# kaist-ina/stellatrain

Measured on AMD Instinct MI355X. Metric: grad-codec GB/s (dense fp32 in) per GPU; thresholdv16 k=1% on 64 MiB bucket, higher is better.
Workload: dtype f32; 1 GPU; thresholdv16 k=167772 (1%) on 64 MiB fp32 buckets; step = 64 keys (4096 MiB) per GPU in 16 batched calls of 4, call j on stream j % 4; n=16777216, dst_len=167772, streams=4, parallelism=bucket-sharded x1, no collective

## Files before the change

### include/stg/codec.h

```cpp
#ifndef STG_CODEC_H
#define STG_CODEC_H

#include <stddef.h>
#include <stdint.h>

#ifdef __cplusplus
extern "C" {
#endif

#define STG_OK 0
#define STG_ERR_INVALID (-1)
#define STG_ERR_UNKNOWN (-2)
#define STG_ERR_HIP (-3)
#define STG_ERR_UNSUPPORTED (-4)
#define STG_ERR_DEVICE (-5)

typedef struct stg_codec *stg_codec_t;
typedef struct stg_sgd *stg_sgd_t;
typedef struct stg_adam *stg_adam_t;

int stg_codec_create(const char *method, int device, stg_codec_t *out);
int stg_codec_destroy(stg_codec_t h);
const char *stg_codec_name(stg_codec_t h);

// ... 11 lines not shown
    size_t n;
    uint32_t k;
    uint32_t *d_idx;
    size_t idx_cap;
    float *d_val;
    size_t val_cap;
    int32_t idx_offset;
    uint32_t *d_count;
} stg_bucket_t;

int stg_codec_compress_batch_device(stg_codec_t h, const stg_bucket_t *buckets, size_t nbuckets, void *stream);

int stg_merge_compress_batch_device(stg_codec_t h, const stg_bucket_t *buckets, float *const *d_residuals,
                                    size_t nbuckets, void *stream);

int stg_merge_gather_compress_device(stg_codec_t h, const stg_bucket_t *bucket, float *d_residual,
                                     const float *const *d_grads, int num_gpus, void *stream);

int stg_codec_compress_wire_batch_device(stg_codec_t h, const stg_bucket_t *buckets, const int *flags,
                                         size_t nbuckets, void *stream);

int stg_codec_get_state(stg_codec_t h, const char *key, const void *key_ptr, float *threshold,
                        float *threshold_inc, void *stream);

int stg_codec_set_timing(stg_codec_t h, int enable);
int stg_codec_get_timing(stg_codec_t h, double *ms3, uint64_t *calls);

int stg_codec_debug_words(stg_codec_t h, void *stream, uint32_t *out, int n);

int stg_codec_check(stg_codec_t h);

int stg_scatter_merge_device(const uint32_t *d_idx, const float *d_val, size_t per_rank, int world, size_t n,
                             float *d_dense, uint8_t *d_mark, uint32_t *d_out_idx, float *d_out_val,
                             uint32_t *d_out_count, void *stream);
int stg_scatter_merge_check(void *stream);
int stg_scatter_merge_release(void *stream);

int stg_error_feedback_device(float *d_grad, size_t n, const uint32_t *d_idx, size_t numel, float *d_residual,
                              void *stream);

int stg_sgd_create(int device, float lr, float momentum, float dampening, float weight_decay, int nesterov,
                   int maximize, stg_sgd_t *out);
int stg_sgd_destroy(stg_sgd_t o);
int stg_sgd_optimize_raw_device(stg_sgd_t o, const char *name, float *d_param, uint32_t param_len,
                                const float *d_grad, const uint32_t *d_idx, uint32_t grad_len,
                                const uint32_t *d_grad_len, void *stream);
// ... 86 lines not shown
```

### stellatrain_amd/_capi.py

```python
from __future__ import annotations

import ctypes as C
import os
import re

_HERE = os.path.dirname(os.path.abspath(__file__))
LIB_PATH = os.environ.get("STG_CODEC_LIB") or os.path.join(_HERE, "libstg_codec.so")
HEADER = os.path.join(os.path.dirname(_HERE), "include", "stg", "codec.h")

STG_OK = 0
ERRORS = {-1: "STG_ERR_INVALID", -2: "STG_ERR_UNKNOWN", -3: "STG_ERR_HIP", -4: "STG_ERR_UNSUPPORTED",
          -5: "STG_ERR_DEVICE"}


class CodecError(RuntimeError):

    def __init__(self, code: int, msg: str):
        super().__init__(msg)
        self.code = code


class StgBucket(C.Structure):
    _fields_ = [("key", C.c_char_p), ("d_src", C.c_void_p), ("n", C.c_size_t), ("k", C.c_uint32),
                ("d_idx", C.c_void_p), ("idx_cap", C.c_size_t), ("d_val", C.c_void_p), ("val_cap", C.c_size_t),
# ... 2 lines not shown

class StgRankStream(C.Structure):
    _fields_ = [("d_idx", C.c_void_p), ("d_val", C.c_void_p), ("flag", C.c_int)]


class StgWireRx(C.Structure):
    _fields_ = [("d_idx_in", C.c_void_p), ("d_val_in", C.c_void_p), ("numel", C.c_size_t), ("flag", C.c_int),
                ("d_idx", C.c_void_p), ("d_val", C.c_void_p)]


_lib: C.CDLL | None = None

_SIGS = {
    "stg_codec_create": (C.c_int, [C.c_char_p, C.c_int, C.POINTER(C.c_void_p)]),
    "stg_codec_destroy": (C.c_int, [C.c_void_p]),
    "stg_codec_name": (C.c_char_p, [C.c_void_p]),
    "stg_codec_compress_host": (C.c_int, [C.c_void_p, C.c_char_p, C.c_void_p, C.c_size_t, C.c_uint32, C.c_void_p,
                                          C.c_size_t, C.c_void_p, C.c_size_t, C.c_int32, C.POINTER(C.c_size_t)]),
    "stg_codec_compress_device": (C.c_int, [C.c_void_p, C.c_char_p, C.c_void_p, C.c_size_t, C.c_uint32, C.c_void_p,
                                            C.c_size_t, C.c_void_p, C.c_size_t, C.c_int32, C.c_void_p, C.c_void_p]),
    "stg_codec_compress_batch_device": (C.c_int, [C.c_void_p, C.POINTER(StgBucket), C.c_size_t, C.c_void_p]),
    "stg_codec_get_state": (C.c_int, [C.c_void_p, C.c_char_p, C.c_void_p, C.POINTER(C.c_float),
                                      C.POINTER(C.c_float), C.c_void_p]),
    "stg_codec_check": (C.c_int, [C.c_void_p]),
    "stg_codec_debug_words": (C.c_int, [C.c_void_p, C.c_void_p, C.c_void_p, C.c_int]),
    "stg_codec_set_timing": (C.c_int, [C.c_void_p, C.c_int]),
    "stg_codec_get_timing": (C.c_int, [C.c_void_p, C.POINTER(C.c_double), C.POINTER(C.c_uint64)]),
    "stg_scatter_merge_device": (C.c_int, [C.c_void_p, C.c_void_p, C.c_size_t, C.c_int, C.c_size_t, C.c_void_p,
                                           C.c_void_p, C.c_void_p, C.c_void_p, C.c_void_p, C.c_void_p]),
    "stg_scatter_merge_check": (C.c_int, [C.c_void_p]),
    "stg_scatter_merge_release": (C.c_int, [C.c_void_p]),
    "stg_error_feedback_device": (C.c_int, [C.c_void_p, C.c_size_t, C.c_void_p, C.c_size_t, C.c_void_p, C.c_void_p]),
    "stg_sgd_create": (C.c_int, [C.c_int, C.c_float, C.c_float, C.c_float, C.c_float, C.c_int, C.c_int,
                                 C.POINTER(C.c_void_p)]),
    "stg_sgd_destroy": (C.c_int, [C.c_void_p]),
    "stg_sgd_optimize_raw_device": (C.c_int, [C.c_void_p, C.c_char_p, C.c_void_p, C.c_uint32, C.c_void_p,
                                              C.c_void_p, C.c_uint32, C.c_void_p, C.c_void_p]),
    "stg_sgd_get_momentum": (C.c_int, [C.c_void_p, C.c_char_p, C.c_void_p, C.c_uint32, C.c_void_p]),
    "stg_sgd_set_smart_momentum": (C.c_int, [C.c_void_p, C.c_int]),
    "stg_sgd_get_last": (C.c_int, [C.c_void_p, C.c_char_p, C.c_void_p, C.c_uint32, C.c_void_p]),
    "stg_sgd_get_iter": (C.c_int, [C.c_void_p, C.POINTER(C.c_uint32)]),
    "stg_sgd_check": (C.c_int, [C.c_void_p, C.c_void_p]),
    "stg_merge_optimize_sgd_device": (C.c_int, [C.c_void_p, C.c_char_p, C.c_void_p, C.c_uint32, C.c_void_p,
                                                C.c_void_p, C.c_size_t, C.c_int, C.c_void_p, C.c_void_p,
                                                C.c_void_p, C.c_void_p, C.c_void_p, C.c_void_p]),
    "stg_merge_optimize_adam_device": (C.c_int, [C.c_void_p, C.c_char_p, C.c_void_p, C.c_uint32, C.c_void_p,
# ... 68 lines not shown
```

### stellatrain_amd/compressor.py

```python
from __future__ import annotations

import ctypes as C

import numpy as np

from ._capi import CodecError, StgBucket, check, lib

__all__ = ["Compressor", "ThresholdvCompressor16", "ThresholdvCompressor", "TopkCompressor", "make_compressor",
           "CodecError"]


def _is_torch(x) -> bool:
    return type(x).__module__.startswith("torch")


def _stream_ptr(device: int) -> int:
    import torch
    return torch.cuda.current_stream(device).cuda_stream


class Compressor:

    _method = ""

# ... 131 lines not shown
    def _compress_host(self, name, src, k, dst_idx, dst_val, idx_offset) -> int:
        s = src.numpy() if _is_torch(src) else src
        di = dst_idx.numpy() if _is_torch(dst_idx) else dst_idx
        dv = dst_val.numpy() if _is_torch(dst_val) else dst_val
        if not (isinstance(s, np.ndarray) and s.dtype == np.float32 and s.flags.c_contiguous):
            raise TypeError("src must be a contiguous float32 array/tensor")
        if di.dtype.itemsize != 4 or dv.dtype != np.float32 or not di.flags.c_contiguous or not dv.flags.c_contiguous:
            raise TypeError("dst_idx must be contiguous (u)int32 and dst_val contiguous float32")
        out = C.c_size_t()
        check(lib().stg_codec_compress_host(
            self._h, name.encode(), C.c_void_p(s.ctypes.data), s.size, int(k), C.c_void_p(di.ctypes.data),
            di.size, C.c_void_p(dv.ctypes.data), dv.size, int(idx_offset), C.byref(out)))
        return int(out.value)

    def state(self, name: str = "", key_ptr: int = 0, stream=None):
        t, inc = C.c_float(), C.c_float()
        sp = stream if stream is not None else 0
        rc = lib().stg_codec_get_state(self._h, name.encode(), C.c_void_p(key_ptr), C.byref(t), C.byref(inc),
                                       C.c_void_p(sp))
        if rc != 0:
            return None
        return t.value, inc.value

    def set_timing(self, enable: bool) -> None:
        check(lib().stg_codec_set_timing(self._h, int(enable)))

    def get_timing(self):
        ms = (C.c_double * 3)()
        calls = C.c_uint64()
        check(lib().stg_codec_get_timing(self._h, ms, C.byref(calls)))
        return (ms[0], ms[1], ms[2]), int(calls.value)

    def check_device(self) -> None:
        check(lib().stg_codec_check(self._h))


class ThresholdvCompressor16(Compressor):

    _method = "thresholdv16"

    def __init__(self, thread_pool=None, multicore: bool = True, *, device: int = 0):
        self.multicore_ = multicore
        super().__init__(thread_pool, device=device)


class ThresholdvCompressor(Compressor):
# ... 27 lines not shown
```

### stellatrain_amd/csrc/capi.cpp

```cpp
#include <cmath>
#include <hip/hip_runtime.h>

#include <algorithm>
#include <array>
#include <map>
#include <cstdio>
#include <cstdlib>
#include <cstring>
#include <memory>
#include <mutex>
#include <string>
#include <unordered_map>
#include <vector>

#include <dlfcn.h>

#include "../../include/stg/codec.h"
#include "ws.h"

namespace {

thread_local std::string g_err;

int fail(int code, const std::string &msg) {
// ... 360 lines not shown
        if (lc <= stg::LMAXC && (rc = ws->ensure_lone(lc))) return rc;
    }
    std::array<hipEvent_t, 3> evs{};
    bool timed = false;
    if ((rc = h->take_events(&evs, &timed))) return rc;
    if (++ws->epoch >= (1u << 24)) {
        ws->epoch = 1;
        HIP_TRY(hipMemsetAsync(ws->d.ctl, 0, sizeof(stg::FillCtl), s));
        HIP_TRY(hipMemsetAsync(ws->d.desc, 0, ws->cap_desc * sizeof(stg::ChunkDesc), s));
    }
    stg::Tv16Launch a{};
    a.b = grp.data();
    a.nb = (uint32_t)grp.size();
    a.num_cu = h->num_cu;
    a.ev = timed ? evs.data() : nullptr;
    a.epoch = ws->epoch;
    const uint32_t inflight = fused_inflight();
    constexpr uint32_t XCDS = 8;
    a.max_wg = (uint32_t)(2 * h->num_cu);
    (void)XCDS;
    a.desc_cap = (uint32_t)std::min<size_t>(ws->cap_desc, 0xffffffffu);
    a.lone_cap = (uint32_t)ws->cap_lone;
    a.lone_calls = &ws->lone_calls;
    if (!inflight) {
        HIP_TRY(stg::launch_tv16(a, ws->d, s));
        grp.clear();
        return STG_OK;
    }
    FusedLane &lane = g_lanes[h->device & 63];
    std::lock_guard<std::mutex> lg(lane.mu);
    const size_t max_inflight = inflight;
    while (lane.inflight.size() >= max_inflight) {
        auto old = lane.inflight.front();
        lane.inflight.erase(lane.inflight.begin());
        if (old.second != s) HIP_TRY(hipStreamWaitEvent(s, old.first, 0));
        lane.pool.push_back(old.first);
    }
    HIP_TRY(stg::launch_tv16(a, ws->d, s));
    hipEvent_t done;
    if (!lane.pool.empty()) { done = lane.pool.back(); lane.pool.pop_back(); }
    else HIP_TRY(hipEventCreateWithFlags(&done, hipEventDisableTiming));
    HIP_TRY(hipEventRecord(done, s));
    lane.inflight.emplace_back(done, s);
    grp.clear();
    return STG_OK;
}
// ... 397 lines not shown
        snprintf(b, sizeof b, "device failure flags 0x%x (details: stg_codec_check)", ws->pinned_count[1]);
        return fail(STG_ERR_DEVICE, b);
    }
    *out_count = *ws->pinned_count;
    return STG_OK;
}

int stg_codec_get_state(stg_codec_t h, const char *key, const void *key_ptr, float *threshold, float *threshold_inc,
                        void *stream) {
    if (!h) return fail(STG_ERR_INVALID, "null codec handle");
    HIP_TRY(hipSetDevice(h->device));
    KeyState *st = nullptr;
    {
        std::lock_guard<std::mutex> g(h->mu);
        auto it = h->slot_of.find(state_key(h->method, key, key_ptr));
        if (it == h->slot_of.end()) return fail(STG_ERR_INVALID, "key has no state yet");
        st = h->slot_ptr(it->second);
    }
    HIP_TRY(hipStreamSynchronize(static_cast<hipStream_t>(stream)));
    KeyState hs;
    HIP_TRY(hipMemcpy(&hs, st, sizeof hs, hipMemcpyDeviceToHost));
    if (threshold) *threshold = hs.t;
    if (threshold_inc) *threshold_inc = hs.inc;
    return STG_OK;
}

int stg_codec_set_timing(stg_codec_t h, int enable) {
    if (!h) return fail(STG_ERR_INVALID, "null codec handle");
    std::lock_guard<std::mutex> g(h->mu);
    h->timing = enable != 0;
    return STG_OK;
}

int stg_codec_get_timing(stg_codec_t h, double *ms3, uint64_t *calls) {
    if (!h || !ms3 || !calls) return fail(STG_ERR_INVALID, "null argument");
    HIP_TRY(hipSetDevice(h->device));
    std::lock_guard<std::mutex> g(h->mu);
    for (auto &e : h->ev_pending) {
        HIP_TRY(hipEventSynchronize(e[2]));
        float a = 0, b = 0, c = 0;
        HIP_TRY(hipEventElapsedTime(&a, e[0], e[1]));
        HIP_TRY(hipEventElapsedTime(&b, e[1], e[2]));
        HIP_TRY(hipEventElapsedTime(&c, e[0], e[2]));
        h->ms_acc[0] += a;
        h->ms_acc[1] += b;
        h->ms_acc[2] += c;
// ... 725 lines not shown
```

### stellatrain_amd/csrc/tv16.hip

```cpp
#include <algorithm>
#include <cstdlib>

#include "tv16_dev.h"

namespace stg {

namespace {

using namespace tv16;
constexpr uint32_t kEfAux = 2;

constexpr uint32_t kTv16Ns = 11;
constexpr uint32_t FWG = (kTv16Ns + 1) * 64;
constexpr uint32_t FNW = FWG / 64;
constexpr uint32_t NS = kTv16Ns;
constexpr uint32_t FIN = NS;
static_assert(NS + 1 <= FNW && FWG <= 1024, "streaming group + finisher fit the workgroup");
constexpr uint32_t kTv16Nbuf = 5;
constexpr uint32_t kTv16ScanD = 3;
constexpr uint32_t NBUF = kTv16Nbuf;
constexpr uint32_t CIDR = 2 * NBUF;
constexpr uint32_t kTv16StageB = 72;
constexpr uint32_t kTv16WlB = 64;
constexpr uint32_t STAGE_B = kTv16StageB;
constexpr uint32_t WL_B = kTv16WlB;
constexpr uint32_t kTv16PollSleep = 8;
constexpr uint32_t GB = 512;
constexpr uint32_t SCAN_D_BATCH = kTv16ScanD;
constexpr uint32_t kTv16ScanDLone = 6;
constexpr uint32_t SCAN_D_LONE = kTv16ScanDLone;
constexpr uint32_t MAXG = 512;
__global__ void __launch_bounds__(STG_WG) tv16_seq_sums(const float *__restrict__ src, size_t n,
                                                        float *__restrict__ out, uint32_t nblk) {
    const uint32_t j = blockIdx.x * STG_WG + threadIdx.x;
    if (j >= nblk) return;
    const size_t base = (size_t)j * 16;
    const uint32_t len = (uint32_t)std::min<size_t>(16, n - base);
    float s = 0.f;
    if (len == 16) {
        const float4 *p = reinterpret_cast<const float4 *>(src + base);
        const float4 a = p[0], b = p[1], c = p[2], d = p[3];
        s += fabsf(a.x); s += fabsf(a.y); s += fabsf(a.z); s += fabsf(a.w);
        s += fabsf(b.x); s += fabsf(b.y); s += fabsf(b.z); s += fabsf(b.w);
        s += fabsf(c.x); s += fabsf(c.y); s += fabsf(c.z); s += fabsf(c.w);
        s += fabsf(d.x); s += fabsf(d.y); s += fabsf(d.z); s += fabsf(d.w);
    } else {
// ... 13 lines not shown
struct BucketDesc {
    const float *src;
    uint32_t *idx;
    float *val;
    uint32_t *count_out;
    KeyState *state;
    float *sums_g;
    uint32_t nb, tl, dst_len;
    int32_t idx_offset;
    uint32_t cs, nc;
    float *resid;
    uint32_t wflag, wend;
};

struct BatchArgs {
    BucketDesc bk[MAX_BATCH];
    uint32_t nbk;
    uint32_t epoch;
    uint32_t K;
    FillCtl *ctl;
    ChunkDesc *desc;
    uint32_t *cand;
    uint32_t *fail;
};

struct Lds {
    float4 stage[NBUF][STAGE_B * 4];
    uint32_t stage_line[NBUF][STAGE_B];
    uint64_t wl[NBUF][WL_B];
    uint32_t nst[NBUF];
    uint32_t nwl[NBUF];
    uint32_t qcnt[NBUF];
    uint32_t wcnt[NBUF];
    uint32_t sdone[NBUF];
    float tval[NBUF], incv[NBUF];
    uint32_t cid[CIDR];
    uint32_t cok[CIDR];
    uint32_t mid[CIDR];
    uint32_t fdone;
    uint4 gb[GB];
};
static_assert(sizeof(Lds) <= TV16_SCAN_LDS, "two scan workgroups and a fill workgroup share a CU");

__device__ __forceinline__ constexpr uint32_t spin_site(uint32_t site) { return FAIL_SPIN_TIMEOUT | (1u << (8 + site)); }

struct Ctx {
    const BatchArgs &A;
    Lds &L;
    uint32_t G, w;
    FillCtl *ctlp;
    uint32_t *candp;
    uint32_t *failp;

    __device__ __forceinline__ uint32_t tag(uint32_t kind) const { return (A.epoch << 8) | kind; }
    __device__ __forceinline__ FillCtl *ctl() const { return ctlp; }
    __device__ __forceinline__ CallCtl *cc() const { return &ctlp->cc[A.epoch & 1u]; }
    __device__ __forceinline__ uint32_t *cand(uint32_t b) const { return candp + (size_t)b * CAND_WORDS; }
    __device__ __forceinline__ void fail(uint32_t bits) const { g_or(failp, bits); }
    __device__ __forceinline__ void spin_fail(uint32_t site, uint32_t x0, uint32_t x1, uint32_t x2) const {
        g_or(failp, spin_site(site));
        if (atomicCAS(failp + 1, 0u, site + 1u) == 0u) {
            st_sc1(failp + 2, w);
            st_sc1(failp + 3, x0);
            st_sc1(failp + 4, x1);
            st_sc1(failp + 5, x2);
            st_sc1(failp + 6, A.epoch);
        }
        uint32_t *rec = failp + 8 + 4 * site;
        if (atomicCAS(rec, 0u, w + 1u) == 0u) {
            st_sc1(rec + 1, x0);
            st_sc1(rec + 2, x1);
            st_sc1(rec + 3, x2);
        }
        for (uint32_t b = 0; b < A.nbk; ++b) st_sc1(A.bk[b].count_out, POISON_COUNT);
    }
    __device__ __forceinline__ uint32_t bucket_of(uint32_t k) const {
        uint32_t b = 0;
        while (b + 1 < A.nbk && k >= A.bk[b + 1].cs) ++b;
        return b;
    }
};

constexpr uint32_t TAG_AGG = 1, TAG_DEC = TV16_TAG_DEC;
constexpr uint32_t DEC_B = TV16_DEC_B, DEC_WIN = TV16_DEC_WIN, DEC_TAIL = TV16_DEC_TAIL;
constexpr uint32_t WIN = TV16_WIN;

template <int STAGE, bool EF, uint32_t SCAN_D>
__device__ __forceinline__ void scan_chunk(Ctx &C, uint32_t j, uint32_t k, uint32_t s) {
    Lds &L = C.L;
    const uint32_t par = j % NBUF;
    if (j >= NBUF) {
        uint64_t st2 = 0;
        uint32_t spins = 0;
        for (; lds_ld(&L.fdone) < j + 1 - NBUF; ++spins) {
            __builtin_amdgcn_s_sleep(2);
            if (spin_expired(spins, st2)) { if (flane() == 0) C.spin_fail(1, j, lds_ld(&L.fdone), s); break; }
        }
    }
    const uint32_t b = C.bucket_of(k);
    const BucketDesc &d = C.A.bk[b];
    const uint32_t c = k - d.cs;
    const uint32_t L0 = c * TV16_CHUNK;
    const uint32_t nl = d.nb > L0 ? std::min(TV16_CHUNK, d.nb - L0) : 0u;
    const float t = uni(d.state->t);
    const uint32_t lane = flane(), q = lane & 3;
    if (s == 0 && lane == 0) { L.tval[par] = t; L.incv[par] = uni(d.state->inc); }
    const uint32_t tb = f2u(t);
    const uint32_t wlo = tb > WIN ? tb - WIN : 0u;
    const uint32_t steps = (nl + 15) / 16;
    const uint32_t mine = steps > s ? (steps - s + NS - 1) / NS : 0u;
    uint32_t cnt_w = 0, win_w = 0;
    const __amdgpu_buffer_rsrc_t rsrc = __builtin_amdgcn_make_buffer_rsrc(
        const_cast<float *>(d.src + (size_t)L0 * 16), 0, nl * 64u, 0x00020000);
    const uint32_t lane_line = s * 16 + (lane >> 2);
    const __amdgpu_buffer_rsrc_t rsrc_r = __builtin_amdgcn_make_buffer_rsrc(
        EF ? d.resid + (size_t)L0 * 16 : nullptr, 0, (EF && d.resid) ? nl * 64u : 0u, 0x00020000);
    auto store_r = [&](uint32_t m, float4 x) {
        uint32_t voff = lane_line * 64u + q * 16u;
        asm volatile("" : "+v"(voff));
        u4v t4;
        t4.x = __float_as_uint(x.x); t4.y = __float_as_uint(x.y); t4.z = __float_as_uint(x.z); t4.w = __float_as_uint(x.w);
        __builtin_amdgcn_raw_buffer_store_b128(t4, rsrc_r, voff + m * (NS * 1024u), 0, kEfAux );
    };
    auto load = [&](uint32_t m) -> float4 {
        uint32_t voff = lane_line * 64u + q * 16u;
        asm volatile("" : "+v"(voff));
        const u4v t4 = __builtin_amdgcn_raw_buffer_load_b128(rsrc, voff + m * (NS * 1024u), 0, 2 );
        return make_float4(__uint_as_float(t4.x), __uint_as_float(t4.y), __uint_as_float(t4.z),
                           __uint_as_float(t4.w));
    };
    float4 v[SCAN_D];
// ... 18 lines not shown
            const uint32_t i = (m0 + u) * (NS * 16u) + ll;
            if (STAGE == 3) {
                cnt_w += f2u(x.x + x.y + x.z + x.w) == 0x7f800001u;
                v[u] = load(m0 + u + SCAN_D);
                continue;
            }
            const float S = quad_line_sum(x);
            if (EF) store_r(m0 + u, x);
            v[u] = load(m0 + u + SCAN_D);
            const uint32_t us = f2u(S);
            const bool near = i < nl && us >= wlo;
            if (!__ballot(near && q == 0)) continue;
            const bool qual = near && S >= t;
            const bool win = near && us < tb;
            const uint64_t bq = __ballot(qual && q == 0);
            const uint64_t bw = __ballot(win && q == 0);
            if (bw) {
                win_w += (uint32_t)__popcll(bw);
                uint32_t base = 0;
                if (lane == 0) base = atomicAdd(&L.nwl[par], (uint32_t)__popcll(bw));
                base = __builtin_amdgcn_readfirstlane(base);
                if (win && q == 0) {
                    const uint32_t slot = base + (uint32_t)__popcll(bw & below_mask(flane()));
                    if (slot < WL_B) L.wl[par][slot] = ((uint64_t)us << 32) | ((L0 + i) * 16);
                }
            }
            if (bq) {
                cnt_w += (uint32_t)__popcll(bq);
                uint32_t base = 0;
                if (lane == 0) base = atomicAdd(&L.nst[par], (uint32_t)__popcll(bq));
                base = __builtin_amdgcn_readfirstlane(base);
                if (qual) {
                    const uint64_t b3 = bq << 3;
                    const uint32_t slot = base + __builtin_amdgcn_mbcnt_hi(
                        (uint32_t)(b3 >> 32), __builtin_amdgcn_mbcnt_lo((uint32_t)b3, 0u));
                    if (slot < STAGE_B) {
                        const uint32_t lq = flane() & 3u;
                        L.stage[par][slot * 4 + lq] = x;
                        if (lq == 0) L.stage_line[par][slot] = i;
                    }
                }
            }
        }
    }
    if (!tried) try_take();
    if (grab && flane() == 0) {
        L.mid[(j + NBUF) % CIDR] = 0;
// ... 71 lines not shown
}

template <int STAGE>
__device__ __forceinline__ void finish_chunk(Ctx &C, uint32_t j, uint32_t k) {
    Lds &L = C.L;
    const uint32_t par = j % NBUF;
    const uint32_t lane = flane();
    uint64_t st5 = 0;
    for (uint32_t spins = 0; lds_ld(&L.sdone[par]) < NS; ++spins) {
        __builtin_amdgcn_s_sleep(1);
        if (spin_expired(spins, st5)) { if (lane == 0) C.spin_fail(3, j, lds_ld(&L.sdone[par]), k); break; }
    }
    if (STAGE == 1 || STAGE == 3) {
        release(C, par, j);
        return;
    }
    const uint32_t b = C.bucket_of(k);
    const BucketDesc &d = C.A.bk[b];
    const uint32_t c = k - d.cs;
    const uint32_t L0 = c * TV16_CHUNK;
    const uint32_t nl = d.nb > L0 ? std::min(TV16_CHUNK, d.nb - L0) : 0u;
    const uint32_t qw = uni(L.qcnt[par]);
    const float t = uni(L.tval[par]), inc = uni(L.incv[par]);

    uint32_t P = 0, Wbef = 0;
    if (c) prefix_counts(C, b, c, P, Wbef);
    const uint32_t ww = uni(L.wcnt[par]);

    const uint32_t kb = d.dst_len / 16, r = d.dst_len % 16;
    const uint32_t lim = kb + (r ? 1u : 0u);
    const bool vec = aligned16(d);
    if (P < lim && qw) {
        if (qw <= STAGE_B) {
            const uint32_t q = lane & 3;
            for (uint32_t e0 = 0; e0 < qw; e0 += 16) {
                const uint32_t e = e0 + (lane >> 2);
                if (e >= qw) continue;
                const uint32_t i = L.stage_line[par][e];
                uint32_t g = P;
                for (uint32_t x = 0; x < qw; ++x) g += L.stage_line[par][x] < i;
                if (g >= lim) continue;
                const uint32_t pos = (L0 + i) * 16 + 4 * q;
                const uint32_t len = g == kb ? r : 16u;
                const uint32_t off = 16 * g + 4 * q;
                const float4 x = L.stage[par][e * 4 + q];
                const uint32_t bi = pos + (uint32_t)d.idx_offset;
// ... 4 lines not shown
#pragma unroll
                    for (uint32_t cc = 0; cc < 4; ++cc) {
                        if (4 * q + cc < len) {
                            put_pair(d, off + cc, bi + cc, xs[cc]);
                        }
                    }
                }
            }
        } else {
            uint32_t base = P;
            for (uint32_t i0 = 0; i0 < nl && base < lim; i0 += 64) {
                const uint32_t i = i0 + lane;
                const bool f = i < nl && lane_line_sum(d.src + (size_t)(L0 + i) * 16) >= t;
                const uint64_t m = __ballot(f);
                if (f) {
                    const uint32_t g = base + (uint32_t)__popcll(m & below_mask(lane));
                    if (g < lim) emit_line(d, vec, (L0 + i) * 16, 16 * g, g == kb ? r : 16u);
                }
                base += (uint32_t)__popcll(m);
            }
        }
    }

    if (Wbef + ww + 1 <= CAND_CAP) {
        const uint32_t nwl = uni(lds_ld(&L.nwl[par]));
        uint32_t *cu = C.cand(b);
        uint32_t *cp = cu + CAND_CAP, *ci = cu + 2 * CAND_CAP;
        const uint32_t tb = f2u(t);
        if (nwl <= WL_B && qw <= STAGE_B) {
            static_assert(WL_B == 64, "one listed entry per lane");
            const uint64_t e = lane < nwl ? L.wl[par][lane] : ~0ull;
            const uint32_t mypos = (uint32_t)e;
            const uint32_t li = mypos / 16 - L0;
            uint32_t before = 0, qb = 0;
            for (uint32_t l = 0; l < nwl; ++l) before += (uint32_t)L.wl[par][l] < mypos;
            for (uint32_t x = 0; x < qw; ++x) qb += L.stage_line[par][x] < li;
            if (lane < nwl) {
                const uint32_t idx = Wbef + before;
                st_sc1(&cu[idx], (uint32_t)(e >> 32));
                st_sc1(&cp[idx], mypos);
                st_sc1(&ci[idx], L0 + li - P - qb);
            }
        } else {
            const uint32_t wlo = tb > WIN ? tb - WIN : 0u;
            uint32_t base = Wbef, qb = P;
            for (uint32_t i0 = 0; i0 < nl; i0 += 64) {
                const uint32_t i = i0 + lane;
                const float S = i < nl ? lane_line_sum(d.src + (size_t)(L0 + i) * 16) : 0.f;
                const uint32_t u = f2u(S);
                const bool qf = i < nl && S >= t;
                const bool wf = i < nl && u >= wlo && u < tb;
                const uint64_t mq = __ballot(qf), mw = __ballot(wf);
                if (wf) {
                    const uint32_t idx = base + (uint32_t)__popcll(mw & below_mask(lane));
                    st_sc1(&cu[idx], u);
                    st_sc1(&cp[idx], (L0 + i) * 16);
                    st_sc1(&ci[idx], L0 + i - (qb + (uint32_t)__popcll(mq & below_mask(lane))));
                }
                base += (uint32_t)__popcll(mw);
                qb += (uint32_t)__popcll(mq);
            }
        }
    }
    release(C, par, j);

    if (c + 1 == d.nc) {
        const uint32_t Qtot = P + qw, Wtot = Wbef + ww;
        const uint32_t c0 = Qtot >= lim ? d.dst_len : 16u * Qtot;
        bool tail_cand = false;
        float tail_key = 0.f;
        uint32_t ct = 0;
        if (c0 < d.dst_len && d.tl) {
            const float *tp = d.src + (size_t)d.nb * 16;
            float s = 0.f;
            for (uint32_t i = 0; i < d.tl; ++i) s += tp[i];
            s = uni(s);
            if (s * 16.0f >= t * (float)d.tl) ct = std::min(d.dst_len - c0, d.tl);
            else { tail_cand = true; tail_key = s * 16.0f / (float)d.tl; }
        }
        const uint32_t cnt = c0 + ct;
        const bool regimeB = cnt < d.dst_len;
        if (lane == 0) {
            if (ct) {
                const size_t p0 = (size_t)d.nb * 16;
                for (uint32_t i = 0; i < ct; ++i) {
                    put_pair(d, c0 + i, (uint32_t)(p0 + i) + (uint32_t)d.idx_offset, d.src[p0 + i]);
                }
            }
            d.state->t = regimeB ? (float)((double)t * 0.99) : t + inc;
            d.state->inc = inc;
            d.state->init = 1;
            st_sc1(d.count_out, (uint32_t)std::min<uint64_t>(d.dst_len, (uint64_t)d.nb * 16 + d.tl));
            if (ld_sc1(C.failp)) st_sc1(d.count_out, POISON_COUNT);
        }
        const uint32_t ncand = d.nb - Qtot;
        const uint32_t M = regimeB ? std::min((d.dst_len - cnt + 15u) / 16u, ncand) : 0u;
        uint32_t flags = 0;
        if (regimeB) flags = DEC_B | (tail_cand ? DEC_TAIL : 0u) | (Wtot >= M && Wtot + 1 <= CAND_CAP ? DEC_WIN : 0u);
        Decision &D = C.ctl()->dec[b];
        if (lane == 0) {
            st_sc1(&D.w[1], ((uint64_t)cnt << 32) | M);
            st_sc1(&D.w[2], ((uint64_t)Wtot << 32) | __float_as_uint(tail_key));
            st_sc1(&D.w[3], ((uint64_t)Qtot << 32) | __float_as_uint(t));
        }
        vm_drain();
        if (lane == 0) st_sc1(&D.w[0], ((uint64_t)C.tag(TAG_DEC) << 32) | flags);
    }
}

template <int STAGE, bool EF, bool LONE>
__global__ void __launch_bounds__(1024) __attribute__((amdgpu_waves_per_eu(LONE ? 6 : 8, 8)))
tv16_batch(BatchArgs A) {
    __shared__ Lds L;
    Ctx C{A, L, gridDim.x, blockIdx.x, A.ctl, A.cand, A.fail};
    {
        uint32_t *z = reinterpret_cast<uint32_t *>(&A.ctl->cc[(A.epoch + 1) & 1u]);
        constexpr uint32_t words = sizeof(CallCtl) / 4;
        const uint32_t per = (words + C.G - 1) / C.G;
        const uint32_t z0 = C.w * per, z1 = std::min(words, z0 + per);
        for (uint32_t i = z0 + threadIdx.x; i < z1; i += FWG) st_sc1(z + i, 0u);
    }
// ... 109 lines not shown
        f.src = b.src;
        f.idx = b.idx;
        f.val = b.val;
        f.count_out = b.count_out;
        f.nb = d.nb;
        f.tl = d.tl;
        f.dst_len = d.dst_len;
        f.idx_offset = d.idx_offset;
        f.wflag = d.wflag;
        f.wend = d.wend;
        f.cand = ws.cand + (size_t)i * CAND_WORDS;
        f.heap = reinterpret_cast<uint2 *>(b.sums);
    }
    if (K > a.desc_cap) return hipErrorInvalidValue;
    bool ef = false;
    for (uint32_t i = 0; i < a.nb; ++i) ef |= a.b[i].resid != nullptr;
    A.nbk = a.nb;
    A.epoch = a.epoch;
    A.K = K;
    A.ctl = ws.ctl;
    A.desc = ws.desc;
    A.cand = ws.cand;
    A.fail = ws.fail;
    const uint32_t G = std::max<uint32_t>(1, std::min<uint32_t>(std::min<uint32_t>(a.max_wg, K), MAXG));
    const bool lone_scan = lone_ok && a.nb == 1;
    const uint32_t KL = lone_chunks(a.b[0].n);
    if (lone_path) {
        if (a.ev) (void)hipEventRecord(a.ev[0], s);
        LScanArgs L{};
        L.src = a.b[0].src;
        L.nb = A.bk[0].nb;
        L.nc = KL;
        L.state = a.b[0].state;
        L.cp = ws.cp;
        L.resid = a.b[0].resid;
        L.ldesc = ws.ldesc;
        L.lq = ws.lq;
        L.lw = ws.lw;
        L.lv = ws.lv;
        L.whist = ws.whist;
        L.went = ws.went;
        L.zero_next = reinterpret_cast<uint32_t *>(&ws.ctl->cc[(a.epoch + 1) & 1u]);
        uint32_t tag = a.epoch;
        if (a.lone_calls) {
            if (++*a.lone_calls == 0) *a.lone_calls = 2;
            tag = *a.lone_calls;
// ... 107 lines not shown
```

### stellatrain_amd/csrc/tv16fill.hip

```cpp
#ifndef STG_WIRE_EMIT
#define STG_WIRE_EMIT 0
#endif
#include <algorithm>
#include <cstddef>

#include "tv16_dev.h"

namespace stg {

namespace {

using namespace tv16;

constexpr uint32_t FILL_WG = 512;
constexpr uint32_t FNW_F = FILL_WG / 64;
constexpr uint32_t EMAX = 4096;
constexpr uint32_t VCAP = 6144;
constexpr uint32_t POS_LIM = (1u << 20) - 1;
constexpr uint32_t NONE = 0xffffffffu;
constexpr uint32_t NONE13 = 0x1fffu;
constexpr uint32_t CNONE = 0xffffffu;
constexpr uint32_t NBIN = 1024;
constexpr uint32_t NDEP = 20;
constexpr uint32_t PT = EMAX / FILL_WG;
// ... 142 lines not shown
            if (vec && len == 16 && (off & 3u) == 0) {
                put_pair4_w<W>(d, o, bi, x[r]);
            } else {
                for (uint32_t c = 0; c < 4; ++c) {
                    if (4 * q + c < len) {
                        put_pair_w<W>(d, o + c, bi + c, d.src[(size_t)pos + 4 * q + c]);
                    }
                }
            }
        }
    }
}
template <uint32_t K = 5, typename GetPos>
__device__ __forceinline__ void emit_order(const Tv16FillBucket &d, uint32_t cnt, uint32_t rem, uint32_t np, uint32_t tail_rank,
                           GetPos pos_of, uint32_t i_lo = 0, uint32_t i_hi = 0xffffffffu) {
    if (STG_WIRE_EMIT && d.wflag) emit_order_w<K, true>(d, cnt, rem, np, tail_rank, pos_of, i_lo, i_hi);
    else emit_order_w<K, false>(d, cnt, rem, np, tail_rank, pos_of, i_lo, i_hi);
}

template <uint32_t KE, bool LONE, typename GetPos>
__device__ __forceinline__ void emit_all(const Tv16FillBucket &d, uint32_t cnt, uint32_t rem, uint32_t P,
                                         uint32_t tail_rank, GetPos pos_of, uint32_t nhelp, CallCtl *ccp,
                                         uint32_t *order_g, uint32_t ready_tag) {
    if (LONE && nhelp) {
        for (uint32_t i = threadIdx.x; i < P; i += FILL_WG) st_sc1(&order_g[i], pos_of(i));
        __builtin_amdgcn_s_waitcnt(0);
        __syncthreads();
        if (threadIdx.x == 0) {
            st_sc1(&ccp->pad[2], P);
            st_sc1(&ccp->pad[3], tail_rank);
            __builtin_amdgcn_s_waitcnt(0);
            st_sc1(&ccp->pad[1], ready_tag);
        }
        emit_order<KE>(d, cnt, rem, P, tail_rank, pos_of, 0, (P + nhelp) / (nhelp + 1));
    } else {
        emit_order<KE>(d, cnt, rem, P, tail_rank, pos_of);
    }
}

__device__ __forceinline__ uint2 hld(const uint2 *h, uint32_t i) {
    const uint64_t v = ld_sc1(reinterpret_cast<const uint64_t *>(h) + i);
    return make_uint2((uint32_t)v, (uint32_t)(v >> 32));
}
__device__ __forceinline__ void hst(uint2 *h, uint32_t i, uint2 v) {
    st_sc1(reinterpret_cast<uint64_t *>(h) + i, ((uint64_t)v.y << 32) | v.x);
}
__device__ void adjust_heap(uint2 *H, uint32_t hole, uint32_t len, uint2 value) {
// ... 359 lines not shown
    }
    static_assert(PRE * FILL_WG <= CAND_CAP, "prefetch inside the window buffer");
    const uint64_t w0 = ld_sc1(&D.w[0]), w1 = ld_sc1(&D.w[1]), w2 = ld_sc1(&D.w[2]), w3 = ld_sc1(&D.w[3]);
    const uint32_t failed = ld_sc1(A.fail);
    if ((uint32_t)(w0 >> 32) != ((A.epoch << 8) | TV16_TAG_DEC)) {
        if (tid == 0) { g_or(A.fail, FAIL_SPIN_TIMEOUT); st_sc1(d.count_out, POISON_COUNT); }
        return;
    }
    const uint32_t flags = (uint32_t)w0;
    if (!(flags & TV16_DEC_B) || failed) return;
    const uint32_t cnt = (uint32_t)(w1 >> 32), M = (uint32_t)w1;
    const uint32_t Wtot = (uint32_t)(w2 >> 32);
    const float tail_key = u2f((uint32_t)w2);
    const uint32_t Qtot = (uint32_t)(w3 >> 32);
    const float t = u2f((uint32_t)w3);
    const bool tail = (flags & TV16_DEC_TAIL) != 0;
    const uint32_t N = d.nb - Qtot + (tail ? 1u : 0u);
    const uint32_t rem = d.dst_len - cnt;
    if (!M && !tail) return;
    if (A.crew && crew_wants(flags, M, A.mode)) return;
    const uint32_t nhelp = LONE ? A.helpers : 0u;
    CallCtl *const ccp = A.cc;
    const uint32_t tb = f2u(t);
    const uint32_t wlo = tb > TV16_WIN ? tb - TV16_WIN : 0u;
    const bool tail_in = tail && tail_key >= u2f(wlo);
    bool fast = (flags & TV16_DEC_WIN) && N <= POS_LIM && Wtot + (tail_in ? 1u : 0u) > 0 && A.mode != 2u &&
                A.mode != 3u;
    if (!fast && tid == 0) {
        if (!(flags & TV16_DEC_WIN)) atomicAdd(&A.dbg[60], 1u);
        if (N > POS_LIM) atomicAdd(&A.dbg[61], 1u);
    }
    uint32_t *const key = S.u.a.key, *const cix = S.u.a.cix;
    auto kbin = [&](uint32_t kb) -> uint32_t {
        const float k = u2f(kb);
        if (k >= t) return 0u;
        if (!(k > 0.f)) return NBIN - 1;
        return min((tb - 1u - kb) >> 8, NBIN - 1);
    };
    auto okey = [&](uint32_t e) -> uint64_t { return (uint64_t)(~ford(u2f(key[e]))) << 32; };
    auto ksum = [&](uint32_t r) -> float { return u2f(key[S.ord[r]]); };
    uint32_t W = 0, Et = NONE;
    uint32_t *const lines_g = reinterpret_cast<uint32_t *>(d.heap);
    auto line_of = [&](uint32_t i) { return ld_sc1(&lines_g[S.ord[i]]); };
    auto line_lds = [&](uint32_t i) { return S.u.a.line[S.ord[i]]; };
    auto pops = [&](uint32_t &P, uint32_t &tail_rank) {
        for (uint32_t i = tid; i < W; i += FILL_WG)
            if (S.ord[i] == Et) S.flag = i;
        __syncthreads();
        tail_rank = S.flag;
        uint32_t npl = 0;
        for (uint32_t i = tid; i < W; i += FILL_WG) {
            const uint32_t off = 16u * i - (tail_rank < i ? 16u - d.tl : 0u);
            if (off < rem) npl = max(npl, i + 1);
        }
        npl = wave_max(npl);
        if ((tid & 63u) == 0) atomicMax(&S.npop, npl);
        __syncthreads();
        P = S.npop;
    };
    if (tid == 0) { S.flag = NONE; S.nv = 0; S.maxpos = 0; S.npop = 0; S.dmax = 0; S.rn = 0; S.nc = 0; S.nu = 0; S.et = NONE; }
// ... 470 lines not shown
```

### stellatrain_amd/csrc/ws.h

```cpp
#pragma once

#include <hip/hip_runtime.h>
#include <stdint.h>

#include "common.h"

namespace stg {

constexpr uint32_t CAND_CAP = 8192;
constexpr uint32_t CAND_WORDS = 4 * CAND_CAP;
constexpr uint32_t TV16_WIN = 1u << 18;
constexpr uint32_t TV16_SCAN_LDS = 35584;

constexpr uint32_t TV_TILE = 8192;
constexpr uint32_t TOPK_SUP_CAP = 1024;
constexpr uint32_t TOPK_LIST_CAP = 4096;
constexpr uint32_t TOPK_LIST_TILES = 8192;
constexpr uint32_t TV_MAXG = 2048;
constexpr uint32_t TV_SCAP = 4096;

constexpr uint32_t RS_BINS = 2048;
constexpr uint32_t RS_SHARDS = 8;
constexpr uint32_t RS_SH_HIST = 4;

constexpr uint32_t MAX_BATCH = 32;
constexpr uint32_t TV16_CHUNK = 2048;
struct CallCtl {
    uint32_t next;
    uint32_t pad[31];
    uint32_t crew_ticket[32];
    uint32_t crew_done[32];
};
struct alignas(32) Decision {
    uint64_t w[4];
};
constexpr uint32_t TV16_DEC_B = 1, TV16_DEC_WIN = 2, TV16_DEC_TAIL = 4;
constexpr uint32_t TV16_TAG_DEC = 3;
constexpr uint32_t POISON_COUNT = 0xffffffffu;
struct FillCtl {
    CallCtl cc[2];
    Decision dec[MAX_BATCH];
};
struct alignas(16) ChunkDesc {
    uint64_t agg;
    uint64_t pad;
};

struct CallParams {
    float t;
    float inc;
    uint32_t pad[2];
};

struct RSel {
    uint32_t prefix;
    uint32_t mask;
    uint32_t rank;
    uint32_t cnt_gt;
    uint32_t done;
// ... 85 lines not shown
    uint32_t k;
    uint32_t dst_len;
    uint32_t *idx;
    float *val;
    int32_t idx_offset;
    uint32_t *count_out;
    KeyState *state;
    bool first;
    float *sums;
    float *resid;
    const GatherArgs *gather;
    uint32_t wflag;
};
struct Tv16Launch {
    const Tv16Bucket *b;
    uint32_t nb;
    int num_cu;
    hipEvent_t *ev;
    uint32_t epoch;
    uint32_t max_wg;
    uint32_t desc_cap;
    uint32_t lone_cap;
    uint32_t *lone_calls;
};
hipError_t launch_tv16(const Tv16Launch &a, const DevWS &ws, hipStream_t s);
struct Tv16FillBucket {
    const float *src;
    uint32_t *idx;
    float *val;
    uint32_t *count_out;
    uint32_t nb, tl, dst_len;
    int32_t idx_offset;
    const uint32_t *cand;
    uint2 *heap;
    uint32_t wflag, wend;
};
struct Tv16FillArgs {
    Tv16FillBucket bk[MAX_BATCH];
    uint32_t nbk;
    uint32_t epoch;
    const Decision *dec;
    uint32_t *fail;
    uint32_t *dbg;
    uint32_t mode;
    uint32_t crew;
    CrewCtl *crew_ctl;
// ... 197 lines not shown
```

Before: 6222 GB/s.

## Add adaptive per-key candidate window rungs for threshold top-k fill

Replaces the fixed candidate window below the threshold with a three-rung adaptive window stored in per-key state. The window widens when too few candidates fall inside it and narrows after a run of calm calls. Window list entries are packed to 32 bits so the LDS list can double to 128 entries, and the candidate capacity grows to 32768. The aim is to keep the fast windowed fill path taken more often instead of falling back to slower paths. In exchange the code adds bookkeeping, debug counters and a larger candidate buffer, and wider windows mean more candidates to sort.

```diff
diff --git a/include/stg/codec.h b/include/stg/codec.h
--- a/include/stg/codec.h
+++ b/include/stg/codec.h
@@ -57,6 +57,8 @@
 
 int stg_codec_get_state(stg_codec_t h, const char *key, const void *key_ptr, float *threshold,
                         float *threshold_inc, void *stream);
+
+int stg_codec_get_window_rung(stg_codec_t h, const char *key, uint32_t *rung, void *stream);
 
 int stg_codec_set_timing(stg_codec_t h, int enable);
 int stg_codec_get_timing(stg_codec_t h, double *ms3, uint64_t *calls);
diff --git a/stellatrain_amd/_capi.py b/stellatrain_amd/_capi.py
--- a/stellatrain_amd/_capi.py
+++ b/stellatrain_amd/_capi.py
@@ -48,6 +48,7 @@
     "stg_codec_compress_batch_device": (C.c_int, [C.c_void_p, C.POINTER(StgBucket), C.c_size_t, C.c_void_p]),
     "stg_codec_get_state": (C.c_int, [C.c_void_p, C.c_char_p, C.c_void_p, C.POINTER(C.c_float),
                                       C.POINTER(C.c_float), C.c_void_p]),
+    "stg_codec_get_window_rung": (C.c_int, [C.c_void_p, C.c_char_p, C.POINTER(C.c_uint32), C.c_void_p]),
     "stg_codec_check": (C.c_int, [C.c_void_p]),
     "stg_codec_debug_words": (C.c_int, [C.c_void_p, C.c_void_p, C.c_void_p, C.c_int]),
     "stg_codec_set_timing": (C.c_int, [C.c_void_p, C.c_int]),
diff --git a/stellatrain_amd/compressor.py b/stellatrain_amd/compressor.py
--- a/stellatrain_amd/compressor.py
+++ b/stellatrain_amd/compressor.py
@@ -177,6 +177,13 @@
             return None
         return t.value, inc.value
 
+    def window_rung(self, name: str, stream=None):
+        r = C.c_uint32()
+        sp = stream if stream is not None else 0
+        if lib().stg_codec_get_window_rung(self._h, name.encode(), C.byref(r), C.c_void_p(sp)) != 0:
+            return None
+        return int(r.value)
+
     def set_timing(self, enable: bool) -> None:
         check(lib().stg_codec_set_timing(self._h, int(enable)))
 
diff --git a/stellatrain_amd/csrc/capi.cpp b/stellatrain_amd/csrc/capi.cpp
--- a/stellatrain_amd/csrc/capi.cpp
+++ b/stellatrain_amd/csrc/capi.cpp
@@ -406,6 +406,13 @@
     a.desc_cap = (uint32_t)std::min<size_t>(ws->cap_desc, 0xffffffffu);
     a.lone_cap = (uint32_t)ws->cap_lone;
     a.lone_calls = &ws->lone_calls;
+    static const uint32_t force_rung = [] {
+        const char *e = getenv("STG_DEBUG_TV16_RUNG");
+        if (!e || !*e) return 0u;
+        const int x = atoi(e);
+        return x >= 0 && x < (int)stg::TV16_NRUNG ? (uint32_t)x + 1u : 0u;
+    }();
+    a.force_rung = force_rung;
     if (!inflight) {
         HIP_TRY(stg::launch_tv16(a, ws->d, s));
         grp.clear();
@@ -849,6 +856,23 @@
     HIP_TRY(hipMemcpy(&hs, st, sizeof hs, hipMemcpyDeviceToHost));
     if (threshold) *threshold = hs.t;
     if (threshold_inc) *threshold_inc = hs.inc;
+    return STG_OK;
+}
+
+int stg_codec_get_window_rung(stg_codec_t h, const char *key, uint32_t *rung, void *stream) {
+    if (!h || !rung) return fail(STG_ERR_INVALID, "null argument");
+    HIP_TRY(hipSetDevice(h->device));
+    KeyState *st = nullptr;
+    {
+        std::lock_guard<std::mutex> g(h->mu);
+        auto it = h->slot_of.find(state_key(h->method, key, nullptr));
+        if (it == h->slot_of.end()) return fail(STG_ERR_INVALID, "key has no state yet");
+        st = h->slot_ptr(it->second);
+    }
+    HIP_TRY(hipStreamSynchronize(static_cast<hipStream_t>(stream)));
+    KeyState hs;
+    HIP_TRY(hipMemcpy(&hs, st, sizeof hs, hipMemcpyDeviceToHost));
+    *rung = stg::win_rung(hs.pad);
     return STG_OK;
 }
 
diff --git a/stellatrain_amd/csrc/tv16.hip b/stellatrain_amd/csrc/tv16.hip
--- a/stellatrain_amd/csrc/tv16.hip
+++ b/stellatrain_amd/csrc/tv16.hip
@@ -21,7 +21,7 @@
 constexpr uint32_t NBUF = kTv16Nbuf;
 constexpr uint32_t CIDR = 2 * NBUF;
 constexpr uint32_t kTv16StageB = 72;
-constexpr uint32_t kTv16WlB = 64;
+constexpr uint32_t kTv16WlB = 128;
 constexpr uint32_t STAGE_B = kTv16StageB;
 constexpr uint32_t WL_B = kTv16WlB;
 constexpr uint32_t kTv16PollSleep = 8;
@@ -81,18 +81,21 @@
     ChunkDesc *desc;
     uint32_t *cand;
     uint32_t *fail;
+    uint32_t *dbg;
+    uint32_t force_rung;
 };
 
 struct Lds {
     float4 stage[NBUF][STAGE_B * 4];
     uint32_t stage_line[NBUF][STAGE_B];
-    uint64_t wl[NBUF][WL_B];
+    uint32_t wl[NBUF][WL_B];
     uint32_t nst[NBUF];
     uint32_t nwl[NBUF];
     uint32_t qcnt[NBUF];
     uint32_t wcnt[NBUF];
     uint32_t sdone[NBUF];
     float tval[NBUF], incv[NBUF];
+    uint32_t rung[NBUF];
     uint32_t cid[CIDR];
     uint32_t cok[CIDR];
     uint32_t mid[CIDR];
@@ -100,6 +103,7 @@
     uint4 gb[GB];
 };
 static_assert(sizeof(Lds) <= TV16_SCAN_LDS, "two scan workgroups and a fill workgroup share a CU");
+static_assert(TV16_CHUNK <= (1u << 11) && win_ulps(TV16_NRUNG - 1) <= (1u << 20), "a packed window entry: 11 + 20 bits");
 
 __device__ __forceinline__ constexpr uint32_t spin_site(uint32_t site) { return FAIL_SPIN_TIMEOUT | (1u << (8 + site)); }
 
@@ -142,7 +146,6 @@
 
 constexpr uint32_t TAG_AGG = 1, TAG_DEC = TV16_TAG_DEC;
 constexpr uint32_t DEC_B = TV16_DEC_B, DEC_WIN = TV16_DEC_WIN, DEC_TAIL = TV16_DEC_TAIL;
-constexpr uint32_t WIN = TV16_WIN;
 
 template <int STAGE, bool EF, uint32_t SCAN_D>
 __device__ __forceinline__ void scan_chunk(Ctx &C, uint32_t j, uint32_t k, uint32_t s) {
@@ -163,9 +166,11 @@
     const uint32_t nl = d.nb > L0 ? std::min(TV16_CHUNK, d.nb - L0) : 0u;
     const float t = uni(d.state->t);
     const uint32_t lane = flane(), q = lane & 3;
-    if (s == 0 && lane == 0) { L.tval[par] = t; L.incv[par] = uni(d.state->inc); }
+    const uint32_t rung = C.A.force_rung ? win_rung(C.A.force_rung - 1u) : win_rung(uni(d.state->pad));
+    if (s == 0 && lane == 0) { L.tval[par] = t; L.incv[par] = uni(d.state->inc); L.rung[par] = rung; }
     const uint32_t tb = f2u(t);
-    const uint32_t wlo = tb > WIN ? tb - WIN : 0u;
+    const uint32_t win = win_ulps(rung);
+    const uint32_t wlo = tb > win ? tb - win : 0u;
     const uint32_t steps = (nl + 15) / 16;
     const uint32_t mine = steps > s ? (steps - s + NS - 1) / NS : 0u;
     uint32_t cnt_w = 0, win_w = 0;
@@ -230,7 +235,7 @@
                 base = __builtin_amdgcn_readfirstlane(base);
                 if (win && q == 0) {
                     const uint32_t slot = base + (uint32_t)__popcll(bw & below_mask(flane()));
-                    if (slot < WL_B) L.wl[par][slot] = ((uint64_t)us << 32) | ((L0 + i) * 16);
+                    if (slot < WL_B) L.wl[par][slot] = (i << 20) | (tb - 1u - us);
                 }
             }
             if (bq) {
@@ -348,6 +353,7 @@
     const uint32_t nl = d.nb > L0 ? std::min(TV16_CHUNK, d.nb - L0) : 0u;
     const uint32_t qw = uni(L.qcnt[par]);
     const float t = uni(L.tval[par]), inc = uni(L.incv[par]);
+    const uint32_t rung = uni(L.rung[par]);
 
     uint32_t P = 0, Wbef = 0;
     if (c) prefix_counts(C, b, c, P, Wbef);
@@ -398,27 +404,30 @@
         }
     }
 
-    if (Wbef + ww + 1 <= CAND_CAP) {
+    if (P < lim && Wbef + ww + 1 <= CAND_CAP) {
         const uint32_t nwl = uni(lds_ld(&L.nwl[par]));
         uint32_t *cu = C.cand(b);
         uint32_t *cp = cu + CAND_CAP, *ci = cu + 2 * CAND_CAP;
         const uint32_t tb = f2u(t);
         if (nwl <= WL_B && qw <= STAGE_B) {
-            static_assert(WL_B == 64, "one listed entry per lane");
-            const uint64_t e = lane < nwl ? L.wl[par][lane] : ~0ull;
-            const uint32_t mypos = (uint32_t)e;
-            const uint32_t li = mypos / 16 - L0;
-            uint32_t before = 0, qb = 0;
-            for (uint32_t l = 0; l < nwl; ++l) before += (uint32_t)L.wl[par][l] < mypos;
-            for (uint32_t x = 0; x < qw; ++x) qb += L.stage_line[par][x] < li;
-            if (lane < nwl) {
+            static_assert(WL_B == 128, "two listed entries per lane");
+            for (uint32_t s0 = 0; s0 < nwl; s0 += 64) {
+                const uint32_t s = s0 + lane;
+                const uint32_t e = s < nwl ? L.wl[par][s] : ~0u;
+                const uint32_t li = e >> 20;
+                uint32_t before = 0, qb = 0;
+                for (uint32_t l = 0; l < nwl; ++l) before += (L.wl[par][l] >> 20) < li;
+                for (uint32_t x = 0; x < qw; ++x) qb += L.stage_line[par][x] < li;
                 const uint32_t idx = Wbef + before;
-                st_sc1(&cu[idx], (uint32_t)(e >> 32));
-                st_sc1(&cp[idx], mypos);
-                st_sc1(&ci[idx], L0 + li - P - qb);
+                if (s < nwl && idx < CAND_CAP) {
+                    st_sc1(&cu[idx], tb - 1u - (e & 0xfffffu));
+                    st_sc1(&cp[idx], (L0 + li) * 16);
+                    st_sc1(&ci[idx], L0 + li - P - qb);
+                }
             }
         } else {
-            const uint32_t wlo = tb > WIN ? tb - WIN : 0u;
+            const uint32_t win = win_ulps(rung);
+            const uint32_t wlo = tb > win ? tb - win : 0u;
             uint32_t base = Wbef, qb = P;
             for (uint32_t i0 = 0; i0 < nl; i0 += 64) {
                 const uint32_t i = i0 + lane;
@@ -427,8 +436,8 @@
                 const bool qf = i < nl && S >= t;
                 const bool wf = i < nl && u >= wlo && u < tb;
                 const uint64_t mq = __ballot(qf), mw = __ballot(wf);
-                if (wf) {
-                    const uint32_t idx = base + (uint32_t)__popcll(mw & below_mask(lane));
+                const uint32_t idx = base + (uint32_t)__popcll(mw & below_mask(lane));
+                if (wf && idx < CAND_CAP) {
                     st_sc1(&cu[idx], u);
                     st_sc1(&cp[idx], (L0 + i) * 16);
                     st_sc1(&ci[idx], L0 + i - (qb + (uint32_t)__popcll(mq & below_mask(lane))));
@@ -456,6 +465,8 @@
         }
         const uint32_t cnt = c0 + ct;
         const bool regimeB = cnt < d.dst_len;
+        const uint32_t ncand = d.nb - Qtot;
+        const uint32_t M = regimeB ? std::min((d.dst_len - cnt + 15u) / 16u, ncand) : 0u;
         if (lane == 0) {
             if (ct) {
                 const size_t p0 = (size_t)d.nb * 16;
@@ -466,13 +477,17 @@
             d.state->t = regimeB ? (float)((double)t * 0.99) : t + inc;
             d.state->inc = inc;
             d.state->init = 1;
+            if (!C.A.force_rung) {
+                const uint32_t pad = d.state->pad, npad = win_update(pad, regimeB, Wtot, M);
+                if (npad != pad) d.state->pad = npad;
+                if (win_rung(npad) > win_rung(pad)) atomicAdd(&C.A.dbg[47], 1u);
+                if (win_rung(npad) < win_rung(pad)) atomicAdd(&C.A.dbg[46], 1u);
+            }
             st_sc1(d.count_out, (uint32_t)std::min<uint64_t>(d.dst_len, (uint64_t)d.nb * 16 + d.tl));
             if (ld_sc1(C.failp)) st_sc1(d.count_out, POISON_COUNT);
         }
-        const uint32_t ncand = d.nb - Qtot;
-        const uint32_t M = regimeB ? std::min((d.dst_len - cnt + 15u) / 16u, ncand) : 0u;
-        uint32_t flags = 0;
-        if (regimeB) flags = DEC_B | (tail_cand ? DEC_TAIL : 0u) | (Wtot >= M && Wtot + 1 <= CAND_CAP ? DEC_WIN : 0u);
+        uint32_t flags = rung << TV16_DEC_RUNG_SHIFT;
+        if (regimeB) flags |= DEC_B | (tail_cand ? DEC_TAIL : 0u) | (Wtot >= M && Wtot + 1 <= CAND_CAP ? DEC_WIN : 0u);
         Decision &D = C.ctl()->dec[b];
         if (lane == 0) {
             st_sc1(&D.w[1], ((uint64_t)cnt << 32) | M);
@@ -628,6 +643,8 @@
     A.desc = ws.desc;
     A.cand = ws.cand;
     A.fail = ws.fail;
+    A.dbg = ws.misc;
+    A.force_rung = a.force_rung <= TV16_NRUNG ? a.force_rung : 0u;
     const uint32_t G = std::max<uint32_t>(1, std::min<uint32_t>(std::min<uint32_t>(a.max_wg, K), MAXG));
     const bool lone_scan = lone_ok && a.nb == 1;
     const uint32_t KL = lone_chunks(a.b[0].n);
diff --git a/stellatrain_amd/csrc/tv16fill.hip b/stellatrain_amd/csrc/tv16fill.hip
--- a/stellatrain_amd/csrc/tv16fill.hip
+++ b/stellatrain_amd/csrc/tv16fill.hip
@@ -188,7 +188,7 @@
 __device__ __forceinline__ void emit_all(const Tv16FillBucket &d, uint32_t cnt, uint32_t rem, uint32_t P,
                                          uint32_t tail_rank, GetPos pos_of, uint32_t nhelp, CallCtl *ccp,
                                          uint32_t *order_g, uint32_t ready_tag) {
-    if (LONE && nhelp) {
+    if (LONE && nhelp && P <= CAND_CAP) {
         for (uint32_t i = threadIdx.x; i < P; i += FILL_WG) st_sc1(&order_g[i], pos_of(i));
         __builtin_amdgcn_s_waitcnt(0);
         __syncthreads();
@@ -594,7 +594,8 @@
     const uint32_t nhelp = LONE ? A.helpers : 0u;
     CallCtl *const ccp = A.cc;
     const uint32_t tb = f2u(t);
-    const uint32_t wlo = tb > TV16_WIN ? tb - TV16_WIN : 0u;
+    const uint32_t rung = dec_rung(flags), win = win_ulps(rung), bsh = win_bin_shift(rung);
+    const uint32_t wlo = tb > win ? tb - win : 0u;
     const bool tail_in = tail && tail_key >= u2f(wlo);
     bool fast = (flags & TV16_DEC_WIN) && N <= POS_LIM && Wtot + (tail_in ? 1u : 0u) > 0 && A.mode != 2u &&
                 A.mode != 3u;
@@ -607,7 +608,7 @@
         const float k = u2f(kb);
         if (k >= t) return 0u;
         if (!(k > 0.f)) return NBIN - 1;
-        return min((tb - 1u - kb) >> 8, NBIN - 1);
+        return min((tb - 1u - kb) >> bsh, NBIN - 1);
     };
     auto okey = [&](uint32_t e) -> uint64_t { return (uint64_t)(~ford(u2f(key[e]))) << 32; };
     auto ksum = [&](uint32_t r) -> float { return u2f(key[S.ord[r]]); };
diff --git a/stellatrain_amd/csrc/winpolicy.h b/stellatrain_amd/csrc/winpolicy.h
--- /dev/null
+++ b/stellatrain_amd/csrc/winpolicy.h
@@ -0,0 +1,42 @@
+#pragma once
+
+#include <stdint.h>
+
+#if defined(__HIPCC__) || defined(__CUDACC__)
+#define STG_WINPOLICY_HD __host__ __device__
+#else
+#define STG_WINPOLICY_HD
+#endif
+
+namespace stg {
+
+constexpr uint32_t TV16_NRUNG = 3;
+constexpr uint32_t TV16_WIN_CALM = 16;
+constexpr uint32_t TV16_WIN_SLACK = 6;
+
+STG_WINPOLICY_HD inline constexpr uint32_t win_rung(uint32_t pad) {
+    return (pad & 3u) < TV16_NRUNG ? (pad & 3u) : TV16_NRUNG - 1u;
+}
+STG_WINPOLICY_HD inline constexpr uint32_t win_calm(uint32_t pad) { return (pad >> 8) & 0xffu; }
+STG_WINPOLICY_HD inline constexpr uint32_t win_pack(uint32_t rung, uint32_t calm) { return rung | (calm << 8); }
+STG_WINPOLICY_HD inline constexpr uint32_t win_ulps(uint32_t rung) {
+    return rung == 0 ? (1u << 18) : rung == 1 ? (1u << 19) : (3u << 18);
+}
+STG_WINPOLICY_HD inline constexpr uint32_t win_bin_shift(uint32_t rung) { return rung == 0 ? 8u : rung == 1 ? 9u : 10u; }
+static_assert(win_ulps(TV16_NRUNG - 1) < (1u << 20), "a window offset fits 20 bits of a packed list entry");
+static_assert((win_ulps(0) >> win_bin_shift(0)) <= 1024 && (win_ulps(1) >> win_bin_shift(1)) <= 1024 &&
+                  (win_ulps(2) >> win_bin_shift(2)) <= 1024,
+              "1024 bins cover every rung's window");
+
+STG_WINPOLICY_HD inline uint32_t win_update(uint32_t pad, bool regimeB, uint32_t Wtot, uint32_t M) {
+    const uint32_t rung = win_rung(pad);
+    if (!regimeB) return win_pack(rung, win_calm(pad));
+    const uint64_t need = (uint64_t)M + 2u;
+    if (Wtot < need) return win_pack(rung + 1u < TV16_NRUNG ? rung + 1u : rung, 0u);
+    if (rung == 0 || Wtot < TV16_WIN_SLACK * need) return win_pack(rung, 0u);
+    const uint32_t calm = win_calm(pad) + 1u;
+    if (calm >= TV16_WIN_CALM) return win_pack(rung - 1u, 0u);
+    return win_pack(rung, calm);
+}
+
+}
diff --git a/stellatrain_amd/csrc/ws.h b/stellatrain_amd/csrc/ws.h
--- a/stellatrain_amd/csrc/ws.h
+++ b/stellatrain_amd/csrc/ws.h
@@ -4,12 +4,14 @@
 #include <stdint.h>
 
 #include "common.h"
+#include "winpolicy.h"
 
 namespace stg {
 
-constexpr uint32_t CAND_CAP = 8192;
+constexpr uint32_t CAND_CAP = 32768;
 constexpr uint32_t CAND_WORDS = 4 * CAND_CAP;
 constexpr uint32_t TV16_WIN = 1u << 18;
+static_assert(TV16_WIN == win_ulps(0), "rung 0 is the fixed window");
 constexpr uint32_t TV16_SCAN_LDS = 35584;
 
 constexpr uint32_t TV_TILE = 8192;
@@ -35,6 +37,8 @@
     uint64_t w[4];
 };
 constexpr uint32_t TV16_DEC_B = 1, TV16_DEC_WIN = 2, TV16_DEC_TAIL = 4;
+constexpr uint32_t TV16_DEC_RUNG_SHIFT = 8;
+__host__ __device__ constexpr uint32_t dec_rung(uint32_t flags) { return win_rung(flags >> TV16_DEC_RUNG_SHIFT); }
 constexpr uint32_t TV16_TAG_DEC = 3;
 constexpr uint32_t POISON_COUNT = 0xffffffffu;
 struct FillCtl {
@@ -166,6 +170,7 @@
     uint32_t desc_cap;
     uint32_t lone_cap;
     uint32_t *lone_calls;
+    uint32_t force_rung;
 };
 hipError_t launch_tv16(const Tv16Launch &a, const DevWS &ws, hipStream_t s);
 struct Tv16FillBucket {
```

Measured after the change: 6208 GB/s, median of 2. About the same (-0.2%).
